# brendisurfs/Distributed-Backtesting-Exploration

Measured on AMD Instinct MI355X. Metric: bar-evals/sec (symbols x params x bars), higher is better.
Workload: dtype f64+int64; 1 GPU; BASELINE config 2: SMA fast/slow crossover, 5,000 symbols x 2,520 daily bars x 400 params per GPU; symbols_total=5000, symbols_per_gpu=5000, bars=2520, params=400, topk=100, parallelism=dp1 (contiguous symbol shards; exchange: none)

## Files before the change

distributed-backtesting-exploration_amd/csrc/device_common.h:

```cpp
#pragma once
#include <type_traits>

#include "internal.h"

namespace bt {

__host__ __device__ inline uint64_t trade_mix(uint64_t w) {
    const uint64_t z = (w ^ (w >> 29)) * 0xBF58476D1CE4E5B9ULL;
    return z ^ (z >> 32);
}
__host__ __device__ inline uint64_t trade_mix_et(uint32_t e, uint32_t t, bool lg) {
    const uint32_t lo = e ^ (t << 2) ^ (t << 31);
    const uint32_t hi = (t >> 1) ^ (lg ? 0x40000002u : 0u);
    const uint64_t z = (((uint64_t)hi << 32) | lo) * 0xBF58476D1CE4E5B9ULL;
    return z ^ (z >> 32);
}
constexpr int kDstLevels = 6;
constexpr int kKeyStride = kTile + 1;

typedef __int128 i128;
typedef __attribute__((address_space(3))) double lds_f64;

struct __attribute__((aligned(16))) Agg {
    int32_t mx, mn, dd, du;
};

__device__ __forceinline__ Agg agg_one(int32_t x) { return Agg{x, x, 0, 0}; }

__device__ __forceinline__ Agg agg_sel(bool c, const Agg& a, const Agg& b) {
    return Agg{c ? a.mx : b.mx, c ? a.mn : b.mn, c ? a.dd : b.dd, c ? a.du : b.du};
}

__device__ __forceinline__ Agg agg_merge(const Agg& a, const Agg& b) {
    Agg r;
    r.mx = max(a.mx, b.mx);
    r.mn = min(a.mn, b.mn);
    r.dd = max(max(a.dd, b.dd), a.mx - b.mn);
    r.du = max(max(a.du, b.du), b.mx - a.mn);
    return r;
}

__device__ __forceinline__ int dst_row(int a, int b) {
    return __builtin_clz((unsigned)(a ^ b) | 1u) - (32 - kDstLevels);
}
__device__ __forceinline__ const Agg* dst_rowp(const Agg* D, int a, int b) {
    return D - (32 - kDstLevels) * kTile + __builtin_clz((unsigned)(a ^ b) | 1u) * kTile;
}

__device__ __forceinline__ Agg dst_query(const Agg* D, const int32_t* cT, int a, int b) {
    if (a == b) return agg_one(cT[a]);
    const int r = dst_row(a, b);
    return agg_merge(D[r * kTile + a], D[r * kTile + b]);
}

__device__ __forceinline__ Agg dst_query_bf(const Agg* D, int a, int b) {
    const Agg* Dr = dst_rowp(D, a, b);
    return agg_merge(Dr[a], Dr[b]);
}

__device__ __forceinline__ Agg dst_query_w(const Agg* D, int a, int b) {
    const Agg* Dr = dst_rowp(D, a, b);
    const int4 u = *reinterpret_cast<const int4*>(Dr + a);
    const int4 v = *reinterpret_cast<const int4*>(Dr + b);
    asm volatile("" ::"v"(u.x), "v"(u.y), "v"(u.z), "v"(u.w), "v"(v.x), "v"(v.y), "v"(v.z), "v"(v.w));
    return agg_merge(Agg{u.x, u.y, u.z, u.w}, Agg{v.x, v.y, v.z, v.w});
}

constexpr Agg kAggId = {0, 0x7FFFFFFF, 0, 0};

__device__ __forceinline__ int64_t wave_iscan_i64(int64_t x) {
    uint32_t lo = (uint32_t)x, hi = (uint32_t)((uint64_t)x >> 32);
#define BT_DPP_STEP(ctrl, rmask)                                                      \
    {                                                                                 \
        const uint32_t ylo = __builtin_amdgcn_update_dpp(0u, lo, ctrl, rmask, 0xf, false); \
        const uint32_t yhi = __builtin_amdgcn_update_dpp(0u, hi, ctrl, rmask, 0xf, false); \
        const uint64_t r = (((uint64_t)hi << 32) | lo) + (((uint64_t)yhi << 32) | ylo);   \
        lo = (uint32_t)r;                                                             \
        hi = (uint32_t)(r >> 32);                                                     \
    }
    BT_DPP_STEP(0x111, 0xf)
    BT_DPP_STEP(0x112, 0xf)
    BT_DPP_STEP(0x114, 0xf)
    BT_DPP_STEP(0x118, 0xf)
    BT_DPP_STEP(0x142, 0xa)
    BT_DPP_STEP(0x143, 0xc)
#undef BT_DPP_STEP
    return (int64_t)(((uint64_t)hi << 32) | lo);
}

#define BT_S64_CTRLS(X)                                                                   \
    X("row_shr:1 row_mask:0xf bank_mask:0xf bound_ctrl:1")                                \
    X("row_shr:2 row_mask:0xf bank_mask:0xf bound_ctrl:1")                                \
    X("row_shr:4 row_mask:0xf bank_mask:0xf bound_ctrl:1")                                \
    X("row_shr:8 row_mask:0xf bank_mask:0xf bound_ctrl:1")                                \
    X("row_bcast:15 row_mask:0xa bank_mask:0xf")                                          \
    X("row_bcast:31 row_mask:0xc bank_mask:0xf")
__device__ __forceinline__ int64_t wave_iscan_i64_ac(int64_t x) {
    uint32_t lo = (uint32_t)x, hi = (uint32_t)((uint64_t)x >> 32);
#define BT_S64_ONE(ctrl)                                                                   \
    "s_nop 1\n"                                                                            \
    "v_add_co_u32_dpp %0, vcc, %0, %0 " ctrl "\n"                                          \
    "v_addc_co_u32_dpp %1, vcc, %1, %1, vcc " ctrl "\n"
    asm volatile(BT_S64_CTRLS(BT_S64_ONE) "s_nop 1" : "+v"(lo), "+v"(hi) : : "vcc");
#undef BT_S64_ONE
    return (int64_t)(((uint64_t)hi << 32) | lo);
}
__device__ __forceinline__ void wave_iscan2_i64_ac(int64_t& x, int64_t& y) {
    uint32_t xl = (uint32_t)x, xh = (uint32_t)((uint64_t)x >> 32);
    uint32_t yl = (uint32_t)y, yh = (uint32_t)((uint64_t)y >> 32);
#define BT_S64_TWO(ctrl)                                                                   \
    "v_add_co_u32_dpp %0, vcc, %0, %0 " ctrl "\n"                                          \
    "v_addc_co_u32_dpp %1, vcc, %1, %1, vcc " ctrl "\n"                                    \
    "v_add_co_u32_dpp %2, vcc, %2, %2 " ctrl "\n"                                          \
    "v_addc_co_u32_dpp %3, vcc, %3, %3, vcc " ctrl "\n"
    asm volatile("s_nop 1\n" BT_S64_CTRLS(BT_S64_TWO) "s_nop 1"
                 : "+v"(xl), "+v"(xh), "+v"(yl), "+v"(yh) : : "vcc");
#undef BT_S64_TWO
    x = (int64_t)(((uint64_t)xh << 32) | xl);
    y = (int64_t)(((uint64_t)yh << 32) | yl);
}
#undef BT_S64_CTRLS

__device__ __forceinline__ uint32_t wave_iscan_u32(uint32_t x) {
    x += __builtin_amdgcn_update_dpp(0u, x, 0x111, 0xf, 0xf, false);
    x += __builtin_amdgcn_update_dpp(0u, x, 0x112, 0xf, 0xf, false);
    x += __builtin_amdgcn_update_dpp(0u, x, 0x114, 0xf, 0xf, false);
    x += __builtin_amdgcn_update_dpp(0u, x, 0x118, 0xf, 0xf, false);
    x += __builtin_amdgcn_update_dpp(0u, x, 0x142, 0xa, 0xf, false);
    x += __builtin_amdgcn_update_dpp(0u, x, 0x143, 0xc, 0xf, false);
    return x;
}

template <int CTRL>
__device__ __forceinline__ int32_t dpp(int32_t old, int32_t x) {
    int32_t r = (int32_t)__builtin_amdgcn_update_dpp((uint32_t)old, (uint32_t)x, CTRL, 0xf, 0xf, false);
    asm volatile("" : "+v"(r));
    return r;
}

template <int M>
__device__ __forceinline__ int32_t dst_partner(int32_t x, int lane) {
    if constexpr (M == 1) {
        return dpp<0xB1>(0, x);
    } else if constexpr (M == 2) {
        return dpp<0x0F>(0, x);
    } else if constexpr (M == 3) {
        const int32_t hm = dpp<0x141>(0, x);
        const int32_t q3 = dpp<0xFF>(0, hm), q0 = dpp<0x00>(0, hm);
        return (lane & 4) ? q3 : q0;
    } else if constexpr (M == 4) {
        const int32_t r0 = dpp<0x150>(0, x), r15 = dpp<0x15F>(0, x);
        return (lane & 8) ? r0 : r15;
    } else {
        static_assert(M == 5, "six levels for 64-lane tiles");
        const int32_t l0 = (int32_t)__builtin_amdgcn_readlane((uint32_t)x, 0);
        const int32_t l31 = (int32_t)__builtin_amdgcn_readlane((uint32_t)x, 31);
        const int32_t l32 = (int32_t)__builtin_amdgcn_readlane((uint32_t)x, 32);
        const int32_t l63 = (int32_t)__builtin_amdgcn_readlane((uint32_t)x, 63);
        return (lane & 16) ? ((lane & 32) ? l32 : l0) : ((lane & 32) ? l63 : l31);
    }
}

template <int M, bool LDSX = false>
__device__ __forceinline__ Agg dst_partner_agg(const Agg& a, int lane) {
    if constexpr (LDSX && M >= 3) {
        constexpr int half = 1 << (M - 1), grp = 1 << M;
        const int src = (lane & half) ? (lane & ~(grp - 1)) : (lane | (grp - 1));
        return Agg{__builtin_amdgcn_ds_bpermute(src << 2, a.mx), __builtin_amdgcn_ds_bpermute(src << 2, a.mn),
                   __builtin_amdgcn_ds_bpermute(src << 2, a.dd), __builtin_amdgcn_ds_bpermute(src << 2, a.du)};
    }
    return Agg{dst_partner<M>(a.mx, lane), dst_partner<M>(a.mn, lane), dst_partner<M>(a.dd, lane),
               dst_partner<M>(a.du, lane)};
}

template <bool LDSX = false>
__device__ __forceinline__ void dst_build(int32_t c, int lane, Agg* D) {
    if (LDSX) asm volatile("" : "+v"(lane));
    Agg S = agg_one(c), Pp = S;
    D[(kDstLevels - 1) * kTile + lane] = S;
    auto level = [&](auto mtag) {
        constexpr int m = decltype(mtag)::value;
        const bool left = (lane & (1 << (m - 1))) == 0;
        const Agg part = dst_partner_agg<m, LDSX>(agg_sel(left, S, Pp), lane);
        S = agg_sel(left, agg_merge(S, part), S);
        Pp = agg_sel(left, Pp, agg_merge(part, Pp));
        D[(kDstLevels - 1 - m) * kTile + lane] = agg_sel(((lane >> m) & 1) != 0, Pp, S);
    };
    level(std::integral_constant<int, 1>{});
    level(std::integral_constant<int, 2>{});
    level(std::integral_constant<int, 3>{});
    level(std::integral_constant<int, 4>{});
    level(std::integral_constant<int, 5>{});
    static_assert(kDstLevels == 6, "levels 1..5 above");
}

__device__ __forceinline__ int64_t lane63_i64(int64_t x) {
    const uint32_t lo = __builtin_amdgcn_readlane((uint32_t)x, 63);
    const uint32_t hi = __builtin_amdgcn_readlane((uint32_t)((uint64_t)x >> 32), 63);
    return (int64_t)(((uint64_t)hi << 32) | lo);
}

__device__ __forceinline__ void fixed_ret(int32_t c, int32_t cp, int64_t& q, int64_t& q2) {
    const double ret = (double)((int64_t)c - cp) / (double)cp;
    q = (int64_t)rint(ret * 72057594037927936.0);
    const double rr = ret * ret;
    q2 = (int64_t)rint(rr * 72057594037927936.0);
}

__device__ __forceinline__ void wave_add_trades(const Out& out, int ntr) {
    unsigned long long v = (unsigned long long)ntr;
#pragma unroll
    for (int d = 32; d > 0; d >>= 1) v += __shfl_down(v, d, 64);
    if ((threadIdx.x & 63) == 0 && v) atomicAdd(out.n_trades, v);
}

}
```

distributed-backtesting-exploration_amd/csrc/k_sma.hip:

```cpp
#include <algorithm>
#include <cmath>
#include <cstdlib>

#include "lds_layout.h"
#include "plan.h"
#include "tile_common.h"

namespace bt {

namespace {

constexpr int kCmpDepth1 = 2;

struct ScanCarry {
    int64_t P;
    int32_t prevc;
    uint32_t tv;
};

__device__ __forceinline__ int32_t load_close(const int32_t* __restrict__ crow, int B, int t) {
    return t < B ? crow[t] : 0;
}

__device__ __forceinline__ void ring_store(double* ring, int R, int t0, int lane, double v) {
    const int i = (t0 + lane + 1) & (R - 1);
    ring[i] = v;
    const int rb = t0 & (R - 1);
    if (rb == 0 || rb == R - kTile) {
        if (i < kRingMirror) ring[R + i] = v;
    }
}

__device__ __forceinline__ void stage_ring(int32_t c, int B, int t0, int lane, int R, double* ring,
                                           int32_t* cT, int64_t* ql, int32_t* narrow,
                                           ScanCarry& cy) {
    const int t = t0 + lane;
    const bool valid = t < B;
    const int32_t cp = (int32_t)__builtin_amdgcn_update_dpp((uint32_t)cy.prevc, (uint32_t)c,
                                                            0x138, 0xf, 0xf, false);
    const int64_t inc = wave_iscan_i64((int64_t)c);
    ring_store(ring, R, t0, lane, (double)(cy.P + inc));
    cT[lane] = c;
    int64_t q = 0, q2 = 0;
    uint32_t dv = 0;
    if (valid && t >= 1) {
        fixed_ret(c, cp, q, q2);
        dv = (uint32_t)abs(c - cp);
    }
    ql[lane] = wave_iscan_i64(q);
    ql[kTile + lane] = wave_iscan_i64(q2);
    const bool big = __ballot(dv >= (1u << 25)) != 0;
    const uint32_t tvt = __builtin_amdgcn_readlane(wave_iscan_u32(min(dv, 1u << 25)), 63);
    cy.tv = big ? (1u << 31) : min(cy.tv + tvt, 1u << 31);
    if (lane == 0) *narrow = cy.tv < (1u << 30);
    cy.P += lane63_i64(inc);
    cy.prevc = (int32_t)__builtin_amdgcn_readlane((uint32_t)c, 63);
}

__device__ __forceinline__ uint32_t grab_issue(uint32_t* ctr, int lane) {
    uint32_t v = 0;
    if (lane == 0) v = atomicAdd(ctr, (uint32_t)kKeyGrab);
    return v;
}

__device__ __forceinline__ int32_t floor_key(double F, double iw) {
    return (int32_t)(F * iw);
}

__host__ __device__ inline uint32_t key_round_len(int nwp, int nwaves) {
    return (uint32_t)kKeyGrab * ((uint32_t)nwp / kKeyGrab + 1 + (uint32_t)nwaves);
}

struct KeyGroup {
    int32_t W[kKeyGrab];
    double I[kKeyGrab];
};
typedef __attribute__((address_space(4))) const int32_t const_i32;
typedef __attribute__((address_space(4))) const double const_f64;
__device__ __forceinline__ KeyGroup key_group(const int32_t* kwin, const double* krecip,
                                              uint32_t w, int nwp) {
    const uint32_t i = min(w - (uint32_t)kKeyGrab, (uint32_t)(nwp - kKeyGrab));
    const_i32* cw = (const_i32*)kwin + i;
    const_f64* cr = (const_f64*)krecip + i;
    KeyGroup g;
#pragma unroll
    for (int q = 0; q < kKeyGrab; ++q) {
        g.W[q] = cw[q];
        g.I[q] = cr[q];
    }
    return g;
}

__device__ __forceinline__ void stage_keys(int t0, int B, int nwp, int nf, int wmax, int R,
                                           const double* ring, const int32_t* __restrict__ kwin,
                                           const double* __restrict__ krecip, int32_t* K,
                                           uint32_t* ctr, uint32_t round, int nwaves, int lane,
                                           const int32_t* cTr, Agg* Dr) {
    const int t = t0 + lane;
    const double* ringl = ring + lane;
    const double top = ringl[(t0 + 1) & (R - 1)];
    const bool full = t0 + 1 - wmax >= 0 && t0 + kTile <= B;
    const uint32_t base = round * key_round_len(nwp, nwaves);
    uint32_t w = __builtin_amdgcn_readlane(grab_issue(ctr, lane), 0) - base;
    KeyGroup gw = key_group(kwin, krecip, w, nwp);
#pragma unroll 1
    while (w < (uint32_t)(nwp + kKeyGrab)) {
        const uint32_t vn = grab_issue(ctr, lane);
        if (w == 0) {
            dst_build<true>(cTr[lane], lane, Dr);
            w = __builtin_amdgcn_readlane(vn, 0) - base;
            gw = key_group(kwin, krecip, w, nwp);
            continue;
        }
        w -= kKeyGrab;
        int32_t kq[kKeyGrab];
#pragma unroll
        for (int q = 0; q < kKeyGrab; ++q) {
            const double F = top - ringl[(t0 + 1 - gw.W[q]) & (R - 1)];
            kq[q] = floor_key(F, gw.I[q]);
        }
        int32_t* Kw = K + w * kKS + lane;
        if (full) {
#pragma unroll
            for (int q = 0; q < kKeyGrab; ++q) Kw[q * kKS] = kq[q];
        } else {
            const bool tin = t < B;
#pragma unroll
            for (int q = 0; q < kKeyGrab; ++q)
                Kw[q * kKS] = (tin && t + 1 - gw.W[q] >= 0) ? kq[q] : ((int)(w + q) < nf ? -1 : -2);
        }
        w = __builtin_amdgcn_readlane(vn, 0) - base;
        gw = key_group(kwin, krecip, w, nwp);
    }
}

__device__ __forceinline__ void cmp4(uint32_t& l, uint32_t& z, const int4& x, const int4& y) {
    const uint32_t d0 = (uint32_t)(x.x - y.x), d1 = (uint32_t)(x.y - y.y);
    const uint32_t d2 = (uint32_t)(x.z - y.z), d3 = (uint32_t)(x.w - y.w);
    l = __builtin_amdgcn_alignbit(l, d0, 31);
    l = __builtin_amdgcn_alignbit(l, d1, 31);
    l = __builtin_amdgcn_alignbit(l, d2, 31);
    l = __builtin_amdgcn_alignbit(l, d3, 31);
    z = min(min(z, d0), d1);
    z = min(min(z, d2), d3);
}

__device__ __forceinline__ void eq4(uint32_t& e, const int4& x, const int4& y) {
    e = __builtin_amdgcn_alignbit(e, min((uint32_t)(x.x - y.x), 1u) - 1u, 31);
    e = __builtin_amdgcn_alignbit(e, min((uint32_t)(x.y - y.y), 1u) - 1u, 31);
    e = __builtin_amdgcn_alignbit(e, min((uint32_t)(x.z - y.z), 1u) - 1u, 31);
    e = __builtin_amdgcn_alignbit(e, min((uint32_t)(x.w - y.w), 1u) - 1u, 31);
}
__device__ __forceinline__ uint64_t eq_word(const int32_t* k1, const int32_t* k2) {
    const int4* r1 = reinterpret_cast<const int4*>(k1);
    const int4* r2 = reinterpret_cast<const int4*>(k2);
    uint32_t e0 = 0, e1 = 0;
#pragma unroll 1
    for (int v = 0; v < 8; ++v) {
        eq4(e0, r1[v], r2[v]);
        eq4(e1, r1[v + 8], r2[v + 8]);
    }
    return ((uint64_t)__builtin_bitreverse32(e1) << 32) | __builtin_bitreverse32(e0);
}

}

struct SmaAcct {
    int32_t pos, e, ce, sb, ntr, e0;
    int32_t g32, m32, r32;
    int64_t R, gap, mdd;
    uint64_t ps1, ps2, h;
    I96 s1, s2;
    Agg agg;
    int64_t Bq, C, D;
    int32_t carried, x1, px1;
    Agg agg1;
};


template <bool PARITY, bool MERGE = true, bool SEG = false, bool NARROW = false>
__device__ __forceinline__ void sma_close(SmaAcct& a, const Agg& seg, int t, int32_t cx,
                                          bt_trade* tr, int cap) {
    const Agg st = MERGE ? agg_merge(a.agg, seg) : seg;
    if (SEG && MERGE && a.carried) {
        a.x1 = t;
        a.px1 = cx;
        a.agg1 = st;
        a.carried = 0;
        a.ntr++;
        return;
    }
    const bool lg = a.pos > 0;
    const int32_t lo = lg ? st.mn - a.ce : a.ce - st.mx;
    const int32_t hi = lg ? st.mx - a.ce : a.ce - st.mn;
    const int32_t path = lg ? st.dd : st.du;
    const int32_t pnl = lg ? cx - a.ce : a.ce - cx;
    if (SEG) {
        const int64_t A0 = -a.R, B0 = a.Bq;
        a.C = max(a.C, A0 - (int64_t)lo);
        a.D = max(a.D, max(B0 - (int64_t)lo, (int64_t)path));
        a.Bq = max(B0, (int64_t)hi) - pnl;
    } else if (NARROW) {
        a.m32 = max(a.m32, max(a.g32 - lo, path));
        a.g32 = max(a.g32, hi) - pnl;
    } else {
        a.mdd = max(a.mdd, max(a.gap - (int64_t)lo, (int64_t)path));
        a.gap = max(a.gap, (int64_t)hi) - pnl;
    }
    if (NARROW)
        a.r32 += pnl;
    else
        a.R += pnl;
    a.h += trade_mix_et((uint32_t)a.e, (uint32_t)t, lg);
    if (PARITY && a.ntr < cap) {
        bt_trade r;
        r.entry_bar = a.e;
        r.exit_bar = t;
        r.side = a.pos;
        r.pad = 0;
        r.entry_px = a.ce;
        r.exit_px = cx;
        tr[a.ntr] = r;
    }
    a.ntr++;
}

template <bool RESET_AGG = true>
__device__ __forceinline__ void sma_open(SmaAcct& a, int b, int t, int32_t cx, int np) {
    a.e = t;
    a.ce = cx;
    a.sb = b;
    if (RESET_AGG) a.agg = kAggId;
    a.pos = np;
}

template <bool PARITY, bool ONE_TRIP, bool FIRST, bool SEG, bool NARROW>
__device__ __forceinline__ void sma_reverse(SmaAcct& a, uint64_t& F, uint64_t& alt, int t0,
                                            const int32_t* cT, const int64_t* ql, const Agg* D,
                                            bt_trade* tr, int cap) {
    const int b = __builtin_ctzll(F);
    F &= F - 1;
    Agg seg;
    int32_t cx;
    uint64_t qb;
    if (ONE_TRIP) {
        const Agg* Dr = dst_rowp(D, a.sb, b);
        const Agg d1 = Dr[a.sb], d2 = Dr[b];
        cx = cT[b];
        qb = (uint64_t)ql[b];
        asm volatile("" ::"v"(d1.mx), "v"(d1.mn), "v"(d1.dd), "v"(d1.du), "v"(d2.mx),
                     "v"(d2.mn), "v"(d2.dd), "v"(d2.du), "v"(cx), "v"((uint32_t)qb),
                     "v"((uint32_t)(qb >> 32)));
        seg = agg_merge(d1, d2);
    } else {
        seg = dst_query_bf(D, a.sb, b);
        cx = cT[b];
        qb = (uint64_t)ql[b];
    }
    alt = qb - alt;
    sma_close<PARITY, FIRST, SEG, NARROW>(a, seg, t0 + b, cx, tr, cap);
    sma_open<FIRST>(a, b, t0 + b, cx, -a.pos);
}

template <bool PARITY, bool ONE_TRIP, bool SEG, bool NARROW>
__device__ __forceinline__ void sma_flips(SmaAcct& a, uint64_t F, int t0, int bl, uint64_t LONG,
                                          const int32_t* cT, const int64_t* ql, const Agg* D,
                                          bt_trade* tr, int cap) {
    const uint64_t FX = (bl >= 0 && bl < 64) ? (F & (1ULL << bl)) : 0ULL;
    F ^= FX;
    if (a.pos == 0 && F != 0) {
        const int b = __builtin_ctzll(F);
        F &= F - 1;
        const int np = ((LONG >> b) & 1) ? 1 : -1;
        const uint64_t qx = (uint64_t)ql[b];
        a.ps1 += np > 0 ? (uint64_t)0 - qx : qx;
        a.ps2 -= (uint64_t)ql[kTile + b];
        a.e0 = t0 + b;
        sma_open(a, b, t0 + b, cT[b], np);
    }
    uint64_t alt = 0;
    if (F) sma_reverse<PARITY, ONE_TRIP, true, SEG, NARROW>(a, F, alt, t0, cT, ql, D, tr, cap);
    while (F) sma_reverse<PARITY, ONE_TRIP, false, SEG, NARROW>(a, F, alt, t0, cT, ql, D, tr, cap);
    a.ps1 += a.pos > 0 ? (uint64_t)0 - (alt << 1) : alt << 1;
    if (FX) {
        const int b = bl;
        const uint64_t qx = (uint64_t)ql[b];
        sma_close<PARITY, true, SEG, NARROW>(a, dst_query_bf(D, a.sb, b), t0 + b, cT[b], tr, cap);
        a.ps1 += a.pos > 0 ? qx : (uint64_t)0 - qx;
        a.ps2 += (uint64_t)ql[kTile + b];
        a.pos = 0;
    }
}

template <bool PARITY, bool STAMPS, bool ONE_TRIP, bool SEG>
__device__ __forceinline__ void sma_body(const SymDesc* __restrict__ syms,
                                         const int32_t* __restrict__ close, const Grid& g,
                                         const Out& out, int dedicated, const SegArgs& sg,
                                         int fix_seg) {
    extern __shared__ __attribute__((aligned(16))) unsigned char smem[];
    const int nf = g.na, ns = g.nb, nw = nf + ns;
    const int R = g.ring;
    const SmaLds LL = sma_lds_layout(R, nw);
    double* ring = reinterpret_cast<double*>(smem + LL.ring);
    int32_t* keys = reinterpret_cast<int32_t*>(smem + LL.keys);
    Agg* dst = reinterpret_cast<Agg*>(smem + LL.dst);
    int32_t* cts = reinterpret_cast<int32_t*>(smem + LL.ct);
    int64_t* qls = reinterpret_cast<int64_t*>(smem + LL.ql);
    int32_t* nars = reinterpret_cast<int32_t*>(smem + LL.nar);
    uint32_t* ctr = reinterpret_cast<uint32_t*>(smem + LL.ctr);

    const int tid = threadIdx.x;
    const int lane = tid & 63;
    const int wave = __builtin_amdgcn_readfirstlane(tid >> 6);
    const int nwaves = (int)blockDim.x >> 6;
    const bool helper = (tid >> 6) == nwaves - 1;
    const int nparam_threads = dedicated ? (int)blockDim.x - 64 : (int)blockDim.x;
    const SymDesc sd = syms[blockIdx.x];
    const int B = sd.bars;
    const int ntiles = (B + kTile - 1) / kTile;
    const int P = g.n_params;
    const int j = blockIdx.y * nparam_threads + tid;
    const bool active = tid < nparam_threads && j < P;
    const int kf = active ? j % nf : 0;
    const int ks = nf + (active ? j / nf : 0);
    const int p = (kf * ns) + (ks - nf);
    const int32_t* crow = close + sd.off;

    SegRange sr{0, 0, 0, 0, ntiles};
    SmaSegRec* mine = nullptr;
    size_t ipos = 0, npos = 0;
    if (SEG) {
        sr = seg_range(sg, fix_seg, ntiles, g.wmax);
        const size_t per_seg = (size_t)gridDim.x * P;
        ipos = sr.seg * per_seg + (size_t)blockIdx.x * P + p;
        npos = (size_t)sg.G * per_seg;
        mine = reinterpret_cast<SmaSegRec*>(sg.rec) + ipos;
        if (fix_seg > 0) {
            if (!__syncthreads_or(active && sg.pos[ipos] != sg.pos[npos + ipos - per_seg])) return;
            if (tid == 0) atomicAdd(sg.refixed, 1ULL);
        }
    }
    const int T_scan = sr.T_scan, T_walk = sr.T_walk, T_acct = sr.T_acct, T_end = sr.T_end;

    const int nwp = (nw + kKeyGrab - 1) / kKeyGrab * kKeyGrab;
    const uint32_t key_round = key_round_len(nwp, nwaves);
    if (tid == 0) {
        const int i0 = (T_scan * kTile) & (R - 1);
        ring[i0] = 0.0;
        if (i0 == 0) ring[R] = 0.0;
        *ctr = (uint32_t)T_walk * key_round;
    }
    __syncthreads();
    const int32_t wf = g.kwin[kf], ws = g.kwin[ks];
    const int warm = max(wf, ws) - 1;
    const uint32_t fsw = (uint32_t)wf | ((uint32_t)ws << 16);
    int wmin = active ? warm : 0x7fffffff;
#pragma unroll
    for (int o = 32; o > 0; o >>= 1) wmin = min(wmin, __shfl_xor(wmin, o));
    const int kfirst = __builtin_amdgcn_readfirstlane(wmin) >> 6;

    ScanCarry cy{0, (T_scan > 0 && T_scan * kTile - 1 < B) ? crow[T_scan * kTile - 1] : 0};
    if (SEG && helper && T_scan < T_walk) {
        constexpr int kLookAhead = 8;
        int32_t cn[kLookAhead];
#pragma unroll
        for (int u = 0; u < kLookAhead; ++u) cn[u] = load_close(crow, B, (T_scan + u) * kTile + lane);
#pragma unroll 1
        for (int T0 = T_scan; T0 < T_walk; T0 += kLookAhead) {
#pragma unroll
            for (int u = 0; u < kLookAhead; ++u) {
                const int T = T0 + u;
                if (T < T_walk) {
                    const int32_t c = cn[u];
                    cn[u] = load_close(crow, B, (T + kLookAhead) * kTile + lane);
                    const int64_t inc = wave_iscan_i64((int64_t)c);
                    ring[(T * kTile + lane + 1) & (R - 1)] = (double)(cy.P + inc);
                    cy.P += lane63_i64(inc);
                    cy.prevc = (int32_t)__builtin_amdgcn_readlane((uint32_t)c, 63);
                }
            }
        }
        ring[R + lane] = ring[lane];
    }
    int32_t cpre = 0;
    if (helper) {
        const int b0 = T_walk * kTile;
        const int32_t c0 = load_close(crow, B, b0 + lane), c1 = load_close(crow, B, b0 + kTile + lane);
        cpre = load_close(crow, B, b0 + 2 * kTile + lane);
        const int s0 = T_walk % kStages, s1 = (T_walk + 1) % kStages;
        if (T_walk < T_end) stage_ring(c0, B, b0, lane, R, ring, cts + s0 * kTile, qls + s0 * 2 * kTile, nars + s0, cy);
        __syncthreads();
        if (T_walk + 1 < T_end)
            stage_ring(c1, B, b0 + kTile, lane, R, ring, cts + s1 * kTile, qls + s1 * 2 * kTile, nars + s1, cy);
    } else {
        __syncthreads();
    }
    if (T_walk < T_end)
        stage_keys(T_walk * kTile, B, nwp, nf, g.wmax, R, ring, g.kwin, g.krecip,
                   keys + (T_walk & 1) * nwp * kKS, ctr, (uint32_t)T_walk, nwaves, lane,
                   cts + (T_walk % kStages) * kTile, dst + (T_walk % kDstStages) * kDstLevels * kTile);
    __syncthreads();

    SmaAcct a;
    a.pos = a.e = a.ce = a.sb = a.ntr = a.e0 = 0;
    a.g32 = a.m32 = a.r32 = 0;
    a.R = a.gap = a.mdd = 0;
    a.ps1 = a.ps2 = 0;
    a.h = 0;
    a.s1.clear();
    a.s2.clear();
    a.agg = kAggId;
    a.Bq = a.C = a.D = kNegInf;
    a.carried = a.x1 = a.px1 = 0;
    a.agg1 = kAggId;
    int32_t start_pos = 0;
    if (SEG && fix_seg > 0 && active) a.pos = sg.pos[npos + ipos - (size_t)gridDim.x * P];
    auto enter_acct = [&]() {
        start_pos = a.pos;
        a.carried = a.pos != 0;
        a.agg = kAggId;
        a.sb = 0;
        a.R = 0;
        a.Bq = a.C = a.D = kNegInf;
        a.ntr = 0;
        a.h = 0;
        a.s1.clear();
        a.s2.clear();
        a.ps1 = a.ps2 = 0;
        a.e0 = -1;
        a.x1 = -1;
        a.px1 = 0;
        a.agg1 = kAggId;
    };
    if (SEG && T_walk == T_acct) enter_acct();
    bt_trade* tr = nullptr;
    auto result_index = [&]() -> size_t {
        int le = lane;
        asm volatile("" : "+v"(le));
        const int je = blockIdx.y * nparam_threads + wave * 64 + le;
        return (size_t)blockIdx.x * P + (size_t)((je % nf) * ns + je / nf);
    };
    const size_t gi = (size_t)blockIdx.x * P + p;
    if (PARITY && active) tr = out.trades + gi * out.trade_cap;
    const int cap = out.trade_cap;

    constexpr bool stamps = STAMPS;
    uint64_t st_acc[7] = {0, 0, 0, 0, 0, 0, 0};
    uint64_t st_prev = 0;
#define BT_STAMP(i)                                             \
    if (stamps) {                                               \
        const uint64_t now_ = __builtin_amdgcn_s_memtime();     \
        st_acc[i] += now_ - st_prev;                            \
        st_prev = now_;                                         \
    }
    if (stamps) st_prev = __builtin_amdgcn_s_memtime();

    auto tile_step = [&](auto narrow_tag, const int k) __attribute__((always_inline)) {
        constexpr bool NARROW = decltype(narrow_tag)::value;
        const int t0 = k * kTile;
        if (helper && k + 2 < T_end && !BT_ABL(g, 1)) {
            if (!BT_ABL(g, 32)) __builtin_amdgcn_s_setprio(2);
            const int s = (k + 2) % kStages;
            stage_ring(cpre, B, t0 + 2 * kTile, lane, R, ring, cts + s * kTile,
                       qls + s * 2 * kTile, nars + s, cy);
            cpre = load_close(crow, B, t0 + 3 * kTile + lane);
            __builtin_amdgcn_s_setprio(0);
        }
        BT_STAMP(0)
        if (SEG && active && k == T_acct && k != T_walk) enter_acct();
        if (active && k >= kfirst) {
            if (ONE_TRIP) __builtin_amdgcn_s_setprio(1);
            const int s = k % kStages;
            const int32_t* cT = cts + s * kTile;
            const int64_t* ql = qls + s * 2 * kTile;
            const Agg* D = dst + (k % kDstStages) * kDstLevels * kTile;
            const int32_t* K = keys + (k & 1) * nwp * kKS;
            const int4* k1 = reinterpret_cast<const int4*>(K + kf * kKS);
            const int4* k2 = reinterpret_cast<const int4*>(K + ks * kKS);
            uint32_t l0 = 0, l1 = 0, z = ~0u;
            if (!BT_ABL(g, 4)) {
#pragma unroll
                for (int v = 0; v < 16; ++v) {
                    if (v < 8) cmp4(l0, z, k1[v], k2[v]);
                    else cmp4(l1, z, k1[v], k2[v]);
                    if (ONE_TRIP ? ((v % kCmpDepth1) == kCmpDepth1 - 1) : (v & 1))
                        __builtin_amdgcn_sched_barrier(0);
                }
            }
            BT_STAMP(2)
            uint64_t L = ((uint64_t)__builtin_bitreverse32(l1) << 32) | __builtin_bitreverse32(l0);
            const int lastdec = B - 2 - t0;
            const int wb = warm - t0;
            const int bl = B - 1 - t0;
            uint64_t LONG, F;
            if (z != 0 && wb <= 0 && lastdec >= 63) {
                LONG = ~L;
                F = (LONG ^ ((LONG << 1) | (uint64_t)(a.pos == 1))) | (uint64_t)(a.pos == 0);
            } else {
                uint64_t vm = lastdec >= 63 ? ~0ULL : (lastdec < 0 ? 0ULL : ((1ULL << (lastdec + 1)) - 1));
                vm &= wb <= 0 ? ~0ULL : (wb >= 64 ? 0ULL : (~0ULL << wb));
                uint64_t G, T = 0;
                if (z != 0) {
                    G = ~L & vm;
                } else {
                    const uint64_t E = eq_word(K + kf * kKS, K + ks * kKS);
                    G = ~(L | E) & vm;
                    T = E & vm;
                }
                L &= vm;
                while (T) {
                    const int b = __builtin_ctzll(T);
                    T &= T - 1;
                    const int t = t0 + b;
                    const double top = ring[(t + 1) & (R - 1)];
                    const int fw = (int)(fsw & 0xffffu), sw = (int)(fsw >> 16);
                    const int64_t Fs = (int64_t)(top - ring[(t + 1 - fw) & (R - 1)]) * sw;
                    const int64_t Lf = (int64_t)(top - ring[(t + 1 - sw) & (R - 1)]) * fw;
                    G |= (uint64_t)(Fs > Lf) << b;
                    L |= (uint64_t)(Fs < Lf) << b;
                }
                uint64_t SHORT;
                {
                    const uint64_t A = ~L;
                    const uint64_t s1 = A + G;
                    uint64_t cout = s1 < A;
                    const uint64_t sum = s1 + (uint64_t)(a.pos == 1);
                    cout |= sum < s1;
                    LONG = ((sum ^ A ^ G) >> 1) | (cout << 63);
                }
                {
                    const uint64_t A = ~G;
                    const uint64_t s1 = A + L;
                    uint64_t cout = s1 < A;
                    const uint64_t sum = s1 + (uint64_t)(a.pos == -1);
                    cout |= sum < s1;
                    SHORT = ((sum ^ A ^ L) >> 1) | (cout << 63);
                }
                if (bl < 64) {
                    const uint64_t keep = bl <= 0 ? 0ULL : ((1ULL << bl) - 1);
                    LONG &= keep;
                    SHORT &= keep;
                }
                const uint64_t pL = (LONG << 1) | (uint64_t)(a.pos == 1);
                const uint64_t pS = (SHORT << 1) | (uint64_t)(a.pos == -1);
                F = (LONG ^ pL) | (SHORT ^ pS);
            }
            BT_STAMP(3)
            uint64_t Fw = F;
            if (BT_ABL(g, 8)) {
                asm volatile("" ::"v"((uint32_t)Fw), "v"((uint32_t)(Fw >> 32)));
                Fw = 0;
            }
            sma_flips<PARITY, ONE_TRIP, SEG, NARROW>(a, Fw, t0, bl, LONG, cT, ql, D, tr, cap);
            BT_STAMP(4)
            if (a.pos != 0) {
                a.agg = agg_merge(a.agg, dst_query_bf(D, a.sb, kTile - 1));
                a.sb = 0;
                const uint64_t q63 = (uint64_t)ql[kTile - 1];
                a.ps1 += a.pos > 0 ? q63 : (uint64_t)0 - q63;
                a.ps2 += (uint64_t)ql[2 * kTile - 1];
            }
            if ((k & 1) || k + 1 == T_end) {
                a.s1.add((int64_t)a.ps1);
                a.s2.add((int64_t)a.ps2);
                a.ps1 = a.ps2 = 0;
            }
            BT_STAMP(5)
            if (ONE_TRIP) __builtin_amdgcn_s_setprio(0);
        }
        if (k + 1 < T_end && !BT_ABL(g, 2))
            stage_keys(t0 + kTile, B, nwp, nf, g.wmax, R, ring, g.kwin, g.krecip, keys + ((k + 1) & 1) * nwp * kKS,
                       ctr, (uint32_t)(k + 1), nwaves, lane, cts + ((k + 1) % kStages) * kTile,
                       dst + ((k + 1) % kDstStages) * kDstLevels * kTile);
        BT_STAMP(1)
        __syncthreads();
        BT_STAMP(6)
    };
    int k = T_walk;
    if (!SEG && k < T_end) {
        bool nar = __builtin_amdgcn_readfirstlane(nars[k % kStages]) != 0;
        while (nar) {
            const int32_t nn = k + 1 < T_end ? nars[(k + 1) % kStages] : 0;
            tile_step(std::true_type{}, k);
            nar = __builtin_amdgcn_readfirstlane(nn) != 0;
            ++k;
        }
        a.gap = (uint32_t)a.g32;
        a.mdd = (uint32_t)a.m32;
        a.R = a.r32;
    }
    for (; k < T_end; ++k) tile_step(std::false_type{}, k);
#undef BT_STAMP
    if (stamps && lane == 0) {
        unsigned long long* d = out.dbg + (helper ? 8 : 0);
        for (int i = 0; i < 7; ++i) atomicAdd(&d[i], (unsigned long long)st_acc[i]);
        atomicAdd(&d[7], 1ULL);
    }
    if (SEG) {
        if (active) {
            SmaSegRec r;
            r.ntr = a.ntr;
            r.e0 = a.e0;
            r.start_pos = start_pos;
            r.end_pos = a.pos;
            r.end_e = a.carried ? -1 : a.e;
            r.end_ce = a.ce;
            r.x1 = a.x1;
            r.px1 = a.px1;
            const Agg g1 = a.x1 >= 0 ? a.agg1 : a.agg;
            r.agg1[0] = g1.mx;
            r.agg1[1] = g1.mn;
            r.agg1[2] = g1.dd;
            r.agg1[3] = g1.du;
            r.end_agg[0] = a.agg.mx;
            r.end_agg[1] = a.agg.mn;
            r.end_agg[2] = a.agg.dd;
            r.end_agg[3] = a.agg.du;
            r.R = a.R;
            r.B = a.Bq;
            r.C = a.C;
            r.D = a.D;
            r.h = a.h;
            r.s1lo = a.s1.lo;
            r.s1hi = a.s1.hi;
            r.s2lo = a.s2.lo;
            r.s2hi = a.s2.hi;
            *mine = r;
            sg.pos[ipos] = (int8_t)start_pos;
            sg.pos[npos + ipos] = (int8_t)a.pos;
        }
        return;
    }
    if (active) {
        const uint64_t s1lo = a.s1.lo, s2lo = a.s2.lo;
        const int64_t s1hi = a.s1.hi64(), s2hi = a.s2.hi64();
        const double sh = sharpe_fx(s1lo, s1hi, s2lo, s2hi, B, g.sqrt_ann);
        bt_summary r;
        r.n_trades = a.ntr;
        r.status = 0;
        r.pnl = a.R;
        r.mdd = a.mdd;
        r.exposure = a.ntr > 0 ? B - 1 - a.e0 : 0;
        r.sharpe = sh;
        r.hash = a.h;
        const size_t go = result_index();
        out.sum[go] = r;
        out.key[go] = order_key(sh);
        if (out.sums != nullptr) out.sums[go] = bt_sums{s1lo, s1hi, s2lo, s2hi};
    }
    wave_add_trades(out, active ? a.ntr : 0);
}

template <bool PARITY, bool STAMPS, bool ONE_TRIP>
__global__ __launch_bounds__(1024) __attribute__((amdgpu_waves_per_eu(6))) void sma_kernel(
    const SymDesc* __restrict__ syms, const int32_t* __restrict__ close, Grid g, Out out,
    int dedicated) {
    sma_body<PARITY, STAMPS, ONE_TRIP, false>(syms, close, g, out, dedicated, SegArgs{}, 0);
}

template <bool ONE_TRIP>
__global__ __launch_bounds__(1024) void sma_seg_kernel(const SymDesc* __restrict__ syms,
                                                       const int32_t* __restrict__ close, Grid g,
                                                       Out out, int dedicated, SegArgs sg,
                                                       int fix_seg) {
    sma_body<false, false, ONE_TRIP, true>(syms, close, g, out, dedicated, sg, fix_seg);
}

__global__ __launch_bounds__(256) void sma_seg_combine(const SymDesc* __restrict__ syms, int n_sym,
                                                       int P, const SmaSegRec* __restrict__ rec,
                                                       int G, double sqrt_ann, Out out) {
    __shared__ int4 stage[256 * sizeof(SmaSegRec) / sizeof(int4)];
    const size_t i0 = (size_t)blockIdx.x * blockDim.x;
    const size_t i = i0 + threadIdx.x;
    const size_t n = (size_t)n_sym * P;
    const size_t nb = min((size_t)blockDim.x, n - i0);
    constexpr int kPer = sizeof(SmaSegRec) / sizeof(int4);
    int ntr = 0;
    {
        const int s = i < n ? (int)(i / P) : 0;
        int32_t pos = 0, e = 0, ce = 0, e0 = -1;
        Agg agg = kAggId;
        int64_t R = 0, gap = 0, mdd = 0;
        uint64_t h = 0;
        i128 s1 = 0, s2 = 0;
        for (int q = 0; q < G; ++q) {
            __syncthreads();
            const int4* src = reinterpret_cast<const int4*>(rec + (size_t)q * n + i0);
            for (int c = threadIdx.x; c < (int)nb * kPer; c += blockDim.x) stage[c] = src[c];
            __syncthreads();
            if (i >= n) continue;
            const SmaSegRec& r = reinterpret_cast<const SmaSegRec*>(stage)[threadIdx.x];
            ntr += r.ntr;
            R += r.R;
            h += r.h;
            s1 += (i128)(((unsigned __int128)(uint64_t)(int64_t)r.s1hi << 64) | r.s1lo);
            s2 += (i128)(((unsigned __int128)(uint64_t)(int64_t)r.s2hi << 64) | r.s2lo);
            if (e0 < 0) e0 = r.e0;
            const Agg a1 = Agg{r.agg1[0], r.agg1[1], r.agg1[2], r.agg1[3]};
            if (pos != 0) {
                if (r.x1 >= 0) {
                    const Agg st = agg_merge(agg, a1);
                    const bool lg = pos > 0;
                    const int32_t lo = lg ? st.mn - ce : ce - st.mx;
                    const int32_t hi = lg ? st.mx - ce : ce - st.mn;
                    const int32_t path = lg ? st.dd : st.du;
                    const int32_t pnl = lg ? r.px1 - ce : ce - r.px1;
                    mdd = max(mdd, max(gap - (int64_t)lo, (int64_t)path));
                    gap = max(gap, (int64_t)hi) - pnl;
                    R += pnl;
                    h += trade_mix_et((uint32_t)e, (uint32_t)r.x1, lg);
                } else {
                    agg = agg_merge(agg, a1);
                }
            }
            mdd = max(mdd, max(gap + r.C, r.D));
            gap = max(gap - r.R, r.B);
            if (r.end_pos == 0) {
                pos = 0;
            } else if (r.end_e >= 0) {
                pos = r.end_pos;
                e = r.end_e;
                ce = r.end_ce;
                agg = Agg{r.end_agg[0], r.end_agg[1], r.end_agg[2], r.end_agg[3]};
            }
        }
        if (i < n) {
            const int B = syms[s].bars;
            const uint64_t s1lo = (uint64_t)s1, s2lo = (uint64_t)s2;
            const int64_t s1hi = (int64_t)(s1 >> 64), s2hi = (int64_t)(s2 >> 64);
            const double sh = sharpe_fx(s1lo, s1hi, s2lo, s2hi, B, sqrt_ann);
            bt_summary r;
            r.n_trades = ntr;
            r.status = 0;
            r.pnl = R;
            r.mdd = mdd;
            r.exposure = ntr > 0 ? B - 1 - e0 : 0;
            r.sharpe = sh;
            r.hash = h;
            out.sum[i] = r;
            out.key[i] = order_key(sh);
            if (out.sums != nullptr) out.sums[i] = bt_sums{s1lo, s1hi, s2lo, s2hi};
        }
    }
    wave_add_trades(out, ntr);
}

namespace {

template <bool ONE_TRIP>
hipError_t launch_sma_variant(const SymDesc* syms, int32_t n_sym, const int32_t* close,
                              const Grid& g, const Out& out, bool parity, const SegArgs& seg,
                              const LaunchPlan& pl, hipStream_t st) {
    const dim3 grid(n_sym, pl.grid_y), block(pl.block);
    if (pl.G > 1) {
        const dim3 sgrid(n_sym, pl.grid_y, pl.G), fgrid(n_sym, pl.grid_y, 1);
        for (int s = 0; s < pl.G; ++s)
            hipLaunchKernelGGL((sma_seg_kernel<ONE_TRIP>), s == 0 ? sgrid : fgrid, block, pl.lds, st, syms,
                               close, g, out, pl.dedicated, seg, s);
        const size_t n = (size_t)n_sym * g.n_params;
        hipLaunchKernelGGL(sma_seg_combine, dim3((unsigned)((n + 255) / 256)), dim3(256), 0, st, syms, n_sym,
                           g.n_params, reinterpret_cast<const SmaSegRec*>(seg.rec), pl.G, g.sqrt_ann, out);
    } else if (parity) {
        hipLaunchKernelGGL((sma_kernel<true, false, ONE_TRIP>), grid, block, pl.lds, st, syms, close, g, out,
                           pl.dedicated);
    } else {
        hipLaunchKernelGGL((sma_kernel<false, false, ONE_TRIP>), grid, block, pl.lds, st, syms, close, g, out,
                           pl.dedicated);
    }
    return hipGetLastError();
}

}

hipError_t launch_sma(const SymDesc* syms, int32_t n_sym, const int32_t* close, const Grid& g,
                      const Out& out, bool parity, const SegArgs& seg, const LaunchPlan& pl,
                      hipStream_t st) {
    if (n_sym <= 0) return hipSuccess;
#ifdef BT_PROFILING
    if (BT_ABL(g, 64)) {
        hipLaunchKernelGGL((sma_kernel<false, true, false>), dim3(n_sym, pl.grid_y), dim3(pl.block), pl.lds, st,
                           syms, close, g, out, pl.dedicated);
        return hipGetLastError();
    }
#endif
    if (pl.one_trip) return launch_sma_variant<true>(syms, n_sym, close, g, out, parity, seg, pl, st);
    return launch_sma_variant<false>(syms, n_sym, close, g, out, parity, seg, pl, st);
}

}
```

Baseline: 4764 billion bar-evals/s.

## Scale SMA crossover keys by a running close-magnitude shift to gain key precision

Tracks a per-symbol shift derived from the bitwise OR of closing prices and packs it into the per-tile narrow word alongside the narrow flag. The key reciprocal is then scaled by a power of two through exponent bit arithmetic, so the integer floor keys use more of the int32 range. This adds a wave OR-scan, a ballot and extra packing on the helper wave for every staged tile. It looks aimed at letting the compare path stay on a cheaper narrow route or avoid ties, at the cost of extra helper-side work and a changed encoding of the narrow word.

```diff
diff --git a/distributed-backtesting-exploration_amd/csrc/device_common.h b/distributed-backtesting-exploration_amd/csrc/device_common.h
--- a/distributed-backtesting-exploration_amd/csrc/device_common.h
+++ b/distributed-backtesting-exploration_amd/csrc/device_common.h
@@ -128,6 +128,16 @@
     x += __builtin_amdgcn_update_dpp(0u, x, 0x118, 0xf, 0xf, false);
     x += __builtin_amdgcn_update_dpp(0u, x, 0x142, 0xa, 0xf, false);
     x += __builtin_amdgcn_update_dpp(0u, x, 0x143, 0xc, 0xf, false);
+    return x;
+}
+
+__device__ __forceinline__ uint32_t wave_ior_u32(uint32_t x) {
+    x |= __builtin_amdgcn_update_dpp(0u, x, 0x111, 0xf, 0xf, false);
+    x |= __builtin_amdgcn_update_dpp(0u, x, 0x112, 0xf, 0xf, false);
+    x |= __builtin_amdgcn_update_dpp(0u, x, 0x114, 0xf, 0xf, false);
+    x |= __builtin_amdgcn_update_dpp(0u, x, 0x118, 0xf, 0xf, false);
+    x |= __builtin_amdgcn_update_dpp(0u, x, 0x142, 0xa, 0xf, false);
+    x |= __builtin_amdgcn_update_dpp(0u, x, 0x143, 0xc, 0xf, false);
     return x;
 }
 
diff --git a/distributed-backtesting-exploration_amd/csrc/k_sma.hip b/distributed-backtesting-exploration_amd/csrc/k_sma.hip
--- a/distributed-backtesting-exploration_amd/csrc/k_sma.hip
+++ b/distributed-backtesting-exploration_amd/csrc/k_sma.hip
@@ -16,7 +16,20 @@
     int64_t P;
     int32_t prevc;
     uint32_t tv;
+    int32_t sh;
 };
+
+__device__ __forceinline__ int32_t key_scale_of(uint32_t c_or) {
+    return (int32_t)__builtin_clz((c_or & 0x7fffffffu) | 1u) - 1;
+}
+__device__ __forceinline__ void scale_update(ScanCarry& cy, int32_t c) {
+    if (__ballot((uint32_t)c >= (1u << (31 - cy.sh))) != 0) {
+        const uint32_t c_or = __builtin_amdgcn_readlane(wave_ior_u32((uint32_t)c), 63);
+        cy.sh = __builtin_amdgcn_readfirstlane(min(cy.sh, key_scale_of(c_or)));
+    }
+}
+__device__ __forceinline__ bool nar_flag(int32_t w) { return (w & 1) != 0; }
+__device__ __forceinline__ int32_t nar_scale(int32_t w) { return w >> 1; }
 
 __device__ __forceinline__ int32_t load_close(const int32_t* __restrict__ crow, int B, int t) {
     return t < B ? crow[t] : 0;
@@ -31,6 +44,7 @@
     }
 }
 
+template <bool SCALE>
 __device__ __forceinline__ void stage_ring(int32_t c, int B, int t0, int lane, int R, double* ring,
                                            int32_t* cT, int64_t* ql, int32_t* narrow,
                                            ScanCarry& cy) {
@@ -52,7 +66,8 @@
     const bool big = __ballot(dv >= (1u << 25)) != 0;
     const uint32_t tvt = __builtin_amdgcn_readlane(wave_iscan_u32(min(dv, 1u << 25)), 63);
     cy.tv = big ? (1u << 31) : min(cy.tv + tvt, 1u << 31);
-    if (lane == 0) *narrow = cy.tv < (1u << 30);
+    if (SCALE) scale_update(cy, c);
+    if (lane == 0) *narrow = (int32_t)(cy.tv < (1u << 30)) | (cy.sh << 1);
     cy.P += lane63_i64(inc);
     cy.prevc = (int32_t)__builtin_amdgcn_readlane((uint32_t)c, 63);
 }
@@ -65,6 +80,9 @@
 
 __device__ __forceinline__ int32_t floor_key(double F, double iw) {
     return (int32_t)(F * iw);
+}
+__device__ __forceinline__ double key_recip_scaled(double iw, uint32_t s20) {
+    return __builtin_bit_cast(double, __builtin_bit_cast(uint64_t, iw) + ((uint64_t)s20 << 32));
 }
 
 __host__ __device__ inline uint32_t key_round_len(int nwp, int nwaves) {
@@ -91,17 +109,20 @@
     return g;
 }
 
+template <bool SCALE>
 __device__ __forceinline__ void stage_keys(int t0, int B, int nwp, int nf, int wmax, int R,
                                            const double* ring, const int32_t* __restrict__ kwin,
                                            const double* __restrict__ krecip, int32_t* K,
                                            uint32_t* ctr, uint32_t round, int nwaves, int lane,
-                                           const int32_t* cTr, Agg* Dr) {
+                                           const int32_t* cTr, Agg* Dr, const int32_t* nar) {
     const int t = t0 + lane;
+    const int32_t narw = SCALE ? *nar : 0;
     const double* ringl = ring + lane;
     const double top = ringl[(t0 + 1) & (R - 1)];
     const bool full = t0 + 1 - wmax >= 0 && t0 + kTile <= B;
     const uint32_t base = round * key_round_len(nwp, nwaves);
     uint32_t w = __builtin_amdgcn_readlane(grab_issue(ctr, lane), 0) - base;
+    const uint32_t sh20 = (uint32_t)nar_scale(__builtin_amdgcn_readfirstlane(narw)) << 20;
     KeyGroup gw = key_group(kwin, krecip, w, nwp);
 #pragma unroll 1
     while (w < (uint32_t)(nwp + kKeyGrab)) {
@@ -117,7 +138,7 @@
 #pragma unroll
         for (int q = 0; q < kKeyGrab; ++q) {
             const double F = top - ringl[(t0 + 1 - gw.W[q]) & (R - 1)];
-            kq[q] = floor_key(F, gw.I[q]);
+            kq[q] = floor_key(F, SCALE ? key_recip_scaled(gw.I[q], sh20) : gw.I[q]);
         }
         int32_t* Kw = K + w * kKS + lane;
         if (full) {
@@ -313,7 +334,7 @@
     const int lane = tid & 63;
     const int wave = __builtin_amdgcn_readfirstlane(tid >> 6);
     const int nwaves = (int)blockDim.x >> 6;
-    const bool helper = (tid >> 6) == nwaves - 1;
+    const bool helper = wave == nwaves - 1;
     const int nparam_threads = dedicated ? (int)blockDim.x - 64 : (int)blockDim.x;
     const SymDesc sd = syms[blockIdx.x];
     const int B = sd.bars;
@@ -359,10 +380,13 @@
     for (int o = 32; o > 0; o >>= 1) wmin = min(wmin, __shfl_xor(wmin, o));
     const int kfirst = __builtin_amdgcn_readfirstlane(wmin) >> 6;
 
-    ScanCarry cy{0, (T_scan > 0 && T_scan * kTile - 1 < B) ? crow[T_scan * kTile - 1] : 0};
+    constexpr bool kScale = ONE_TRIP || SEG;
+    ScanCarry cy{0, (T_scan > 0 && T_scan * kTile - 1 < B) ? crow[T_scan * kTile - 1] : 0, 0,
+                 kScale ? 30 : 0};
     if (SEG && helper && T_scan < T_walk) {
         constexpr int kLookAhead = 8;
         int32_t cn[kLookAhead];
+        uint32_t cor = 0;
 #pragma unroll
         for (int u = 0; u < kLookAhead; ++u) cn[u] = load_close(crow, B, (T_scan + u) * kTile + lane);
 #pragma unroll 1
@@ -373,6 +397,7 @@
                 if (T < T_walk) {
                     const int32_t c = cn[u];
                     cn[u] = load_close(crow, B, (T + kLookAhead) * kTile + lane);
+                    cor |= (uint32_t)c;
                     const int64_t inc = wave_iscan_i64((int64_t)c);
                     ring[(T * kTile + lane + 1) & (R - 1)] = (double)(cy.P + inc);
                     cy.P += lane63_i64(inc);
@@ -381,6 +406,7 @@
             }
         }
         ring[R + lane] = ring[lane];
+        cy.sh = key_scale_of(__builtin_amdgcn_readlane(wave_ior_u32(cor), 63));
     }
     int32_t cpre = 0;
     if (helper) {
@@ -388,17 +414,18 @@
         const int32_t c0 = load_close(crow, B, b0 + lane), c1 = load_close(crow, B, b0 + kTile + lane);
         cpre = load_close(crow, B, b0 + 2 * kTile + lane);
         const int s0 = T_walk % kStages, s1 = (T_walk + 1) % kStages;
-        if (T_walk < T_end) stage_ring(c0, B, b0, lane, R, ring, cts + s0 * kTile, qls + s0 * 2 * kTile, nars + s0, cy);
+        if (T_walk < T_end) stage_ring<kScale>(c0, B, b0, lane, R, ring, cts + s0 * kTile, qls + s0 * 2 * kTile, nars + s0, cy);
         __syncthreads();
         if (T_walk + 1 < T_end)
-            stage_ring(c1, B, b0 + kTile, lane, R, ring, cts + s1 * kTile, qls + s1 * 2 * kTile, nars + s1, cy);
+            stage_ring<kScale>(c1, B, b0 + kTile, lane, R, ring, cts + s1 * kTile, qls + s1 * 2 * kTile, nars + s1, cy);
     } else {
         __syncthreads();
     }
     if (T_walk < T_end)
-        stage_keys(T_walk * kTile, B, nwp, nf, g.wmax, R, ring, g.kwin, g.krecip,
+        stage_keys<kScale>(T_walk * kTile, B, nwp, nf, g.wmax, R, ring, g.kwin, g.krecip,
                    keys + (T_walk & 1) * nwp * kKS, ctr, (uint32_t)T_walk, nwaves, lane,
-                   cts + (T_walk % kStages) * kTile, dst + (T_walk % kDstStages) * kDstLevels * kTile);
+                   cts + (T_walk % kStages) * kTile, dst + (T_walk % kDstStages) * kDstLevels * kTile,
+                   nars + T_walk % kStages);
     __syncthreads();
 
     SmaAcct a;
@@ -461,7 +488,7 @@
         if (helper && k + 2 < T_end && !BT_ABL(g, 1)) {
             if (!BT_ABL(g, 32)) __builtin_amdgcn_s_setprio(2);
             const int s = (k + 2) % kStages;
-            stage_ring(cpre, B, t0 + 2 * kTile, lane, R, ring, cts + s * kTile,
+            stage_ring<kScale>(cpre, B, t0 + 2 * kTile, lane, R, ring, cts + s * kTile,
                        qls + s * 2 * kTile, nars + s, cy);
             cpre = load_close(crow, B, t0 + 3 * kTile + lane);
             __builtin_amdgcn_s_setprio(0);
@@ -569,20 +596,20 @@
             if (ONE_TRIP) __builtin_amdgcn_s_setprio(0);
         }
         if (k + 1 < T_end && !BT_ABL(g, 2))
-            stage_keys(t0 + kTile, B, nwp, nf, g.wmax, R, ring, g.kwin, g.krecip, keys + ((k + 1) & 1) * nwp * kKS,
+            stage_keys<kScale>(t0 + kTile, B, nwp, nf, g.wmax, R, ring, g.kwin, g.krecip, keys + ((k + 1) & 1) * nwp * kKS,
                        ctr, (uint32_t)(k + 1), nwaves, lane, cts + ((k + 1) % kStages) * kTile,
-                       dst + ((k + 1) % kDstStages) * kDstLevels * kTile);
+                       dst + ((k + 1) % kDstStages) * kDstLevels * kTile, nars + (k + 1) % kStages);
         BT_STAMP(1)
         __syncthreads();
         BT_STAMP(6)
     };
     int k = T_walk;
     if (!SEG && k < T_end) {
-        bool nar = __builtin_amdgcn_readfirstlane(nars[k % kStages]) != 0;
+        bool nar = nar_flag(__builtin_amdgcn_readfirstlane(nars[k % kStages]));
         while (nar) {
             const int32_t nn = k + 1 < T_end ? nars[(k + 1) % kStages] : 0;
             tile_step(std::true_type{}, k);
-            nar = __builtin_amdgcn_readfirstlane(nn) != 0;
+            nar = nar_flag(__builtin_amdgcn_readfirstlane(nn));
             ++k;
         }
         a.gap = (uint32_t)a.g32;
```

Result: no change. 4756 billion bar-evals/s (-0.2%).
